# gduguey/DiffUS

Hardware: AMD Instinct MI355X
Metric: ray-steps/sec fwd+bwd (higher is better)
Workload: dtype f32

## Files before the change

### diffus_amd/csrc/scatter.hip

```cpp
#include "diffus_host.hpp"

namespace {

#ifdef DIFFUS_STAMP
__device__ unsigned long long *g_stamps = nullptr;
#define STAMP(i)                                                                          \
    do {                                                                                  \
        if (threadIdx.x == 0 && g_stamps) g_stamps[((size_t)blockIdx.y * gridDim.x + blockIdx.x) * 8 + (i)] = __builtin_readcyclecounter(); \
    } while (0)
#define STAMPV(i, v)                                                                     \
    do {                                                                                  \
        if (threadIdx.x == 0 && g_stamps) g_stamps[((size_t)blockIdx.y * gridDim.x + blockIdx.x) * 8 + (i)] = (unsigned long long)(v); \
    } while (0)
#define STAMP_NOW() __builtin_readcyclecounter()
#else
#define STAMP(i) ((void)0)
#define STAMPV(i, v) ((void)0)
#define STAMP_NOW() 0ull
#endif

template <int LAYOUT>
__device__ __forceinline__ int tile_unit(int v, int axis)
{
    if (LAYOUT == DIFFUS_CANONICAL) return v;
    return axis == 2 ? (v >> 1) : (v >> 2);
}

#ifndef DIFFUS_SCATTER_THREADS
#define DIFFUS_SCATTER_THREADS 256
#endif
#ifndef DIFFUS_SC_PATCH_STEPS
#define DIFFUS_SC_PATCH_STEPS DIFFUS_PATCH_STEPS
#endif
#ifndef DIFFUS_SC_PATCH_RAYS
#define DIFFUS_SC_PATCH_RAYS DIFFUS_PATCH_RAYS
#endif
#ifndef DIFFUS_SC_MIN_BLOCKS
#define DIFFUS_SC_MIN_BLOCKS 6
#endif
#ifdef DIFFUS_SC_EXIT
#define SC_EXIT(n)                                                                                                      \
    if (DIFFUS_SC_EXIT == (n)) {                                                                                        \
        _Pragma("unroll") for (int q_ = 0; q_ < kSPT; ++q_)                                                             \
            asm volatile("" ::"v"(zb[q_]), "v"(tx[q_]), "v"(ty[q_]), "v"(x0[q_]), "v"(y0[q_]), "v"(x1[q_]), "v"(y1[q_])); \
        return true;                                                                                                    \
    }
#else
#define SC_EXIT(n) ((void)0)
#endif
constexpr int kScRays = DIFFUS_SC_PATCH_RAYS, kScSteps = DIFFUS_SC_PATCH_STEPS;
constexpr int kSB = DIFFUS_SCATTER_THREADS, kSW = kSB / kWave, kSPT = kScRays * kScSteps / kSB;
#ifndef DIFFUS_SLAB_CAP
#define DIFFUS_SLAB_CAP 9216
#endif
#ifndef DIFFUS_SLAB_MIN_BLOCKS
#define DIFFUS_SLAB_MIN_BLOCKS 4
#endif
constexpr int kSlabCap = DIFFUS_SLAB_CAP;
#ifndef DIFFUS_SC_ROW_PAD
#define DIFFUS_SC_ROW_PAD 1
#endif
constexpr unsigned kRowPad = DIFFUS_SC_ROW_PAD;

template <int SAMPLER, int PM, int CAP>
__device__ __forceinline__ bool scatter_patch_planar(const Args &A, double *tile, int (*s_box)[4], int *s_planar, int *s_live, const Pose &ps,
                                                     const float *rows, unsigned row_off, bool ray_ok, int nbase, int tid)
{
    const int wib = tid >> 6;
    constexpr int kCapD = CAP / 2;
    float zb[kSPT];
    {
        const char *rb = reinterpret_cast<const char *>(rows);
#ifdef DIFFUS_ABLATE_SC_LOAD
        if (true) {
#pragma unroll
            for (int q = 0; q < kSPT; ++q) zb[q] = (ray_ok && nbase + q < A.N1) ? 1e-3f * (float)((tid + q) & 15) : 0.f;
        } else
#endif
        if (ray_ok && nbase + kSPT <= A.N1) {
            if constexpr (kSPT == 4) {
                const F4a4 t = *reinterpret_cast<const F4a4 *>(rb + (size_t)row_off);
                zb[0] = t.x; zb[1] = t.y; zb[2] = t.z; zb[3] = t.w;
            } else {
#pragma unroll
                for (int q = 0; q < kSPT; ++q) zb[q] = ldb_f32(rows, row_off + 4u * q);
            }
        } else {
#pragma unroll
            for (int q = 0; q < kSPT; ++q) zb[q] = (ray_ok && nbase + q < A.N1) ? ldb_f32(rows, row_off + 4u * q) : 0.f;
        }
    }
    {
        int4 *t4 = reinterpret_cast<int4 *>(tile);
#pragma unroll
        for (int e = 0; e < CAP / 4 / kSB; ++e) t4[e * kSB + tid] = make_int4(0, 0, 0, 0);
        static_assert(CAP % (4 * kSB) == 0, "tile clear assumes whole int4 passes");
    }
    const bool ray_planar = (PM == 0 || ps.pmode != 2) ? (ps.df[2] == 0.f) : (ps.dd[2] == 0.0);
    const bool wave_planar = __ballot(ray_planar) == ~0ull;
    int x0[kSPT], x1[kSPT], y0[kSPT], y1[kSPT];
    float tx[kSPT], ty[kSPT];
#pragma unroll
    for (int q = 0; q < kSPT; ++q) {
        const float kf = (float)(A.start + nbase + q);
        const float p0 = ray_point_f<PM>(ps, 0, kf), p1 = ray_point_f<PM>(ps, 1, kf);
        if (SAMPLER == DIFFUS_NEAREST) {
            x0[q] = x1[q] = nearest_index(p0, A.G.d0);
            y0[q] = y1[q] = nearest_index(p1, A.G.d1);
            tx[q] = ty[q] = 0.f;
        } else {
            const Axis a = tri_axis(p0, A.G.d0), b = tri_axis(p1, A.G.d1);
            x0[q] = a.i0; x1[q] = a.i1; tx[q] = a.t;
            y0[q] = b.i0; y1[q] = b.i1; ty[q] = b.t;
        }
    }
    const bool has = ray_ok && nbase < A.N1;
    int bx[4];
    bx[0] = has ? min(x0[0], x0[kSPT - 1]) : 0x7fffffff;
    bx[1] = has ? max(x1[0], x1[kSPT - 1]) : -1;
    bx[2] = has ? min(y0[0], y0[kSPT - 1]) : 0x7fffffff;
    bx[3] = has ? max(y1[0], y1[kSPT - 1]) : -1;
    if (tid == 0) *s_live = 0;
    STAMP(1);
    SC_EXIT(1);
    bx[0] = wave_reduce_minmax<true>(bx[0]);
    bx[1] = wave_reduce_minmax<false>(bx[1]);
    bx[2] = wave_reduce_minmax<true>(bx[2]);
    bx[3] = wave_reduce_minmax<false>(bx[3]);
    if ((tid & 63) == 63) {
        s_planar[wib] = wave_planar;
#pragma unroll
        for (int a = 0; a < 4; ++a) s_box[wib][a] = bx[a];
    }
    __syncthreads();
    STAMP(2);
    SC_EXIT(2);
    int wb[kSW][4];
    int all_planar = 1;
#pragma unroll
    for (int wv = 0; wv < kSW; ++wv) {
        all_planar &= s_planar[wv];
#pragma unroll
        for (int a = 0; a < 4; ++a) wb[wv][a] = __builtin_amdgcn_readfirstlane(s_box[wv][a]) >> 2;
    }
    if (!__builtin_amdgcn_readfirstlane(all_planar)) return false;
    auto box_of = [&](int w0, int cnt, int &l0, int &l1, int &b0, int &b1) -> int {
        int mn0 = 0x7fffffff, mx0 = -1, mn1 = 0x7fffffff, mx1 = -1;
#pragma unroll
        for (int wv = 0; wv < kSW; ++wv) {
            const bool in = wv >= w0 && wv < w0 + cnt;
            mn0 = in ? min(mn0, wb[wv][0]) : mn0; mx0 = in ? max(mx0, wb[wv][1]) : mx0;
            mn1 = in ? min(mn1, wb[wv][2]) : mn1; mx1 = in ? max(mx1, wb[wv][3]) : mx1;
        }
        l0 = mn0; l1 = mn1; b0 = mx0 - mn0 + 1; b1 = mx1 - mn1 + 1;
        if (mx0 < 0 || mx1 < 0) return 0;
        const unsigned e0 = (unsigned)min(b0, 0x3fff), e1 = (unsigned)min(b1, 0x3fff);
        return (int)min(4u * e0 * (4u * e1 + kRowPad), (unsigned)kCapD + 1u);
    };
    static_assert(kSW == 4 || kSW == 8, "wave grouping below: 1, 2 or 4 groups of waves");
    int nsub = 1, l0, l1, b0, b1;
    int need = box_of(0, kSW, l0, l1, b0, b1);
    if (need > kCapD) {
        int t0, t1, t2, t3;
        nsub = 2;
        if (box_of(0, kSW / 2, t0, t1, t2, t3) > kCapD || box_of(kSW / 2, kSW / 2, t0, t1, t2, t3) > kCapD) nsub = 4;
    }
    int iz0, iz1;
    float tz;
    {
        const float p2 = ray_point_f<PM>(ps, 2, 0.f);
        if (SAMPLER == DIFFUS_NEAREST) {
            iz0 = iz1 = nearest_index(p2, A.G.d2);
            tz = 0.f;
        } else {
            const Axis c = tri_axis(p2, A.G.d2);
            iz0 = c.i0; iz1 = c.i1; tz = c.t;
        }
        iz0 = __builtin_amdgcn_readfirstlane(iz0); iz1 = __builtin_amdgcn_readfirstlane(iz1);
        tz = __int_as_float(__builtin_amdgcn_readfirstlane(__float_as_int(tz)));
    }
    const int wpg = kSW / nsub;
    {
        unsigned nz = 0;
#pragma unroll
        for (int q = 0; q < kSPT; ++q) {
            if (!finitef(zb[q])) zb[q] = 0.f;
            nz |= __float_as_uint(zb[q]) & 0x7fffffffu;
        }
        if (__builtin_amdgcn_ballot_w64(nz != 0u) != 0ull && (tid & 63) == 63) *s_live = 1;
    }
#pragma unroll 1
    for (int sp = 0; sp < nsub; ++sp) {
        if (nsub > 1) need = box_of(sp * wpg, wpg, l0, l1, b0, b1);
        if (need == 0) continue;
        const bool mine = (wib / wpg) == sp;
#pragma unroll
        for (int q = 0; q < kSPT; ++q)
            asm volatile("" : "+v"(zb[q]), "+v"(tx[q]), "+v"(ty[q]), "+v"(x0[q]), "+v"(y0[q]), "+v"(x1[q]), "+v"(y1[q]));
        if (need > kCapD) {
            if (mine) {
#pragma unroll
                for (int q = 0; q < kSPT; ++q)
                    if (zb[q] != 0.f) {
                        Cell c;
                        c.i0[0] = x0[q]; c.i1[0] = x1[q]; c.t[0] = tx[q];
                        c.i0[1] = y0[q]; c.i1[1] = y1[q]; c.t[1] = ty[q];
                        c.i0[2] = iz0; c.i1[2] = iz1; c.t[2] = tz;
                        for_each_corner<SAMPLER>(c, zb[q], [&](int i, int j, int k, float v) {
                            if (v != 0.f) {
                                unsigned g = vox_off<DIFFUS_BRICKED>(A.G, i, j, k);
                                atomicAdd(A.gvol + g, v);
                                if (A.gtouched) A.gtouched[g >> 5] = 1;
                            }
                        });
                    }
            }
            continue;
        }
        STAMP(3);
    SC_EXIT(3);
        const int BY = 4 * b1 + kRowPad;
        const int org = -(4 * l0) * BY - 4 * l1;
        const int BY8 = BY * 8, org8 = org * 8;
        char *tile_c = reinterpret_cast<char *>(tile);
        auto add_at = [&](int byte_off, double v) { atomicAdd(reinterpret_cast<double *>(tile_c + byte_off), v); };
        if (mine) {
#pragma unroll
        for (int q = 0; q < kSPT; ++q) {
            const bool on = zb[q] != 0.f;
            const int r0 = __mul24(x0[q], BY8) + org8, r1 = __mul24(x1[q], BY8) + org8;
            const int e00 = r0 + 8 * y0[q], e11 = r1 + 8 * y1[q];
            float c00, c01 = 0.f, c10 = 0.f, c11 = 0.f;
            if constexpr (SAMPLER == DIFFUS_NEAREST) {
                c00 = zb[q];
            } else {
                const float wa1 = tx[q], wa0 = 1.f - wa1, wb1 = ty[q], wb0 = 1.f - wb1;
                const float s0 = zb[q] * wa0, s1 = zb[q] * wa1;
                c00 = s0 * wb0; c01 = s0 * wb1; c10 = s1 * wb0; c11 = s1 * wb1;
            }
#ifdef DIFFUS_ABLATE_SC_ADD
            asm volatile("" :: "v"(c00), "v"(c01), "v"(c10), "v"(c11), "v"(e00), "v"(e11));
            continue;
#endif
            const unsigned long long act = __builtin_amdgcn_ballot_w64(on);
            if (act == 0ull) continue;
            const int lead = __builtin_ctzll(act);
            const int f00 = __builtin_amdgcn_readlane(e00, lead), f11 = __builtin_amdgcn_readlane(e11, lead);
            const unsigned long long eq = __builtin_amdgcn_ballot_w64(e00 == f00) & __builtin_amdgcn_ballot_w64(e11 == f11);
            const bool same = (eq & act) == act;
            if (same && __builtin_popcountll(act) > 4) {
                const int f01 = __builtin_amdgcn_readlane(r0 + 8 * y1[q], lead), f10 = __builtin_amdgcn_readlane(r1 + 8 * y0[q], lead);
                const double t00 = wave_sum_to_lane63((double)c00);
                double t01 = 0.0, t10 = 0.0, t11 = 0.0;
                if constexpr (SAMPLER != DIFFUS_NEAREST) {
                    t01 = wave_sum_to_lane63((double)c01);
                    t10 = wave_sum_to_lane63((double)c10);
                    t11 = wave_sum_to_lane63((double)c11);
                }
                if ((tid & 63) == 63) {
                    if (t00 != 0.0) add_at(f00, t00);
                    if (t01 != 0.0) add_at(f01, t01);
                    if (t10 != 0.0) add_at(f10, t10);
                    if (t11 != 0.0) add_at(f11, t11);
                }
            } else {
                if (c00 != 0.f) add_at(e00, (double)c00);
                if constexpr (SAMPLER != DIFFUS_NEAREST) {
                    if (c01 != 0.f) add_at(r0 + 8 * y1[q], (double)c01);
                    if (c10 != 0.f) add_at(r1 + 8 * y0[q], (double)c10);
                    if (c11 != 0.f) add_at(e11, (double)c11);
                }
            }
            __builtin_amdgcn_sched_barrier(0);
        }
        }
        __syncthreads();
        STAMP(4);
    SC_EXIT(4);
        if (__builtin_amdgcn_readfirstlane(*s_live) == 0) continue;
        {
            const int lane = tid & 63, o = lane & 31, h = lane >> 5;
            const int zz = (o & 1) ? iz1 : iz0;
            const float wz = (iz1 == iz0) ? ((o & 1) ? 0.f : 1.f) : ((o & 1) ? tz : 1.f - tz);
            const bool adds = wz != 0.f, h0 = h == 0;
            const unsigned lc_tile = (unsigned)((__mul24(o >> 3, BY) + 4 * h + ((o >> 1) & 3)) * 8);
            const unsigned lc_g = (__umul24((unsigned)h, (unsigned)A.G.nb2) + (unsigned)(zz >> 1)) * kBrickFloats * 4u
                                  + (unsigned)(((o >> 1) << 1) + (zz & 1)) * 4u;
            const unsigned lc_t = (__umul24((unsigned)h, (unsigned)A.G.nb2) + (unsigned)(zz >> 1)) * 4u;
            unsigned lc_tile_o = lc_tile;
            asm volatile("" : "+v"(lc_tile_o));
            const char *tile_b = reinterpret_cast<const char *>(tile);
            const int wv = __builtin_amdgcn_readfirstlane(wib);
            const unsigned nb2u = (unsigned)A.G.nb2;
            char *const gvol_b = reinterpret_cast<char *>(A.gvol);
            char *const gt_b = reinterpret_cast<char *>(A.gtouched);
            auto flush_pair = [&](unsigned trow, unsigned grow, int cp, double &v, unsigned &ta) {
                const bool second = 2 * cp + 1 < b1;
                ta = trow + 64u * (unsigned)cp + lc_tile_o;
                v = (h0 || second) ? *reinterpret_cast<const double *>(tile_b + ta) : 0.0;
                (void)grow;
            };
            auto emit_pair = [&](unsigned grow, int cp, double v, unsigned ta) {
                if (nsub > 1 && v != 0.0 && !(o & 1)) *reinterpret_cast<double *>(const_cast<char *>(tile_b) + ta) = 0.0;
                const bool nz = v != 0.0 && adds;
#ifdef DIFFUS_ABLATE_SC_FLUSH
                asm volatile("" :: "s"(grow), "v"((float)v * wz), "v"(nz));
#else
                if (nz) {
                    const unsigned gb = grow + 2u * (unsigned)cp * nb2u;
                    if (A.gtouched) *reinterpret_cast<int *>(gt_b + (size_t)gb * 4u + (size_t)lc_t) = 1;
                    atomicAdd(reinterpret_cast<float *>(gvol_b + (size_t)gb * (kBrickFloats * 4u) + (size_t)lc_g), (float)v * wz);
                }
#endif
            };
            const int npr = (b1 + 1) >> 1;
            for (int ci = wv >> 1; ci < b0; ci += 2) {
                const unsigned trow = (unsigned)(4 * ci * BY) * 8u;
                const unsigned grow = ((unsigned)(l0 + ci) * (unsigned)A.G.nb1 + (unsigned)l1) * nb2u;
                for (int cp = wv & 1; cp < npr; cp += 4) {
                    double v0, v1 = 0.0;
                    unsigned t0, t1 = 0;
                    const bool two = cp + 2 < npr;
                    flush_pair(trow, grow, cp, v0, t0);
                    if (two) flush_pair(trow, grow, cp + 2, v1, t1);
                    emit_pair(grow, cp, v0, t0);
                    if (two) emit_pair(grow, cp + 2, v1, t1);
                }
            }
        }
        STAMP(5);
#ifdef DIFFUS_STAMP
        if (threadIdx.x == 0 && g_stamps) {
            g_stamps[((size_t)blockIdx.y * gridDim.x + blockIdx.x) * 8 + 6] = (unsigned long long)need;
            g_stamps[((size_t)blockIdx.y * gridDim.x + blockIdx.x) * 8 + 7] = (unsigned long long)nsub;
        }
#endif
        if (sp + 1 < nsub) __syncthreads();
    }
    return true;
}


template <int SAMPLER, int PM, int CAP>
__device__ __forceinline__ void scatter_patch_planar_merged(const Args &A, double *tile, int (*s_box)[4], int *s_planar, int *s_live, const Pose &ps,
                                                            const float *rows, unsigned row_off, bool ray_ok, int nbase, int ng, int tid)
{
    constexpr int kCapD = CAP / 2, kMaxG = 4;
    const int wib = tid >> 6;
    float zb[kMaxG][kSPT];
    {
        const char *rb = reinterpret_cast<const char *>(rows);
#pragma unroll
        for (int g = 0; g < kMaxG; ++g) {
            const int n0 = nbase + g * kScSteps;
            const unsigned off = row_off + (unsigned)(g * kScSteps) * 4u;
            if (g < ng && ray_ok && n0 + kSPT <= A.N1) {
                if constexpr (kSPT == 4) {
                    const F4a4 t = *reinterpret_cast<const F4a4 *>(rb + (size_t)off);
                    zb[g][0] = t.x; zb[g][1] = t.y; zb[g][2] = t.z; zb[g][3] = t.w;
                } else {
#pragma unroll
                    for (int q = 0; q < kSPT; ++q) zb[g][q] = ldb_f32(rows, off + 4u * q);
                }
            } else {
#pragma unroll
                for (int q = 0; q < kSPT; ++q) zb[g][q] = (g < ng && ray_ok && n0 + q < A.N1) ? ldb_f32(rows, off + 4u * q) : 0.f;
            }
        }
    }
    {
        int4 *t4 = reinterpret_cast<int4 *>(tile);
#pragma unroll
        for (int e = 0; e < CAP / 4 / kSB; ++e) t4[e * kSB + tid] = make_int4(0, 0, 0, 0);
    }
    const bool ray_planar = (PM == 0 || ps.pmode != 2) ? (ps.df[2] == 0.f) : (ps.dd[2] == 0.0);
    const bool wave_planar = __ballot(ray_planar) == ~0ull;
    auto cell_xy = [&](int n, int &x0, int &x1, int &y0, int &y1, float &tx, float &ty) {
        const float kf = (float)(A.start + n);
        const float p0 = ray_point_f<PM>(ps, 0, kf), p1 = ray_point_f<PM>(ps, 1, kf);
        if (SAMPLER == DIFFUS_NEAREST) {
            x0 = x1 = nearest_index(p0, A.G.d0); y0 = y1 = nearest_index(p1, A.G.d1);
            tx = ty = 0.f;
        } else {
            const Axis a = tri_axis(p0, A.G.d0), b = tri_axis(p1, A.G.d1);
            x0 = a.i0; x1 = a.i1; tx = a.t; y0 = b.i0; y1 = b.i1; ty = b.t;
        }
    };
    int bx[4];
    {
        int ax0, ax1, ay0, ay1, bx0, bx1, by0, by1;
        float t0, t1;
        cell_xy(nbase, ax0, ax1, ay0, ay1, t0, t1);
        cell_xy(nbase + (ng - 1) * kScSteps + kSPT - 1, bx0, bx1, by0, by1, t0, t1);
        const bool has = ray_ok && nbase < A.N1;
        bx[0] = has ? min(ax0, bx0) : 0x7fffffff; bx[1] = has ? max(ax1, bx1) : -1;
        bx[2] = has ? min(ay0, by0) : 0x7fffffff; bx[3] = has ? max(ay1, by1) : -1;
    }
    if (tid == 0) *s_live = 0;
    bx[0] = wave_reduce_minmax<true>(bx[0]);
    bx[1] = wave_reduce_minmax<false>(bx[1]);
    bx[2] = wave_reduce_minmax<true>(bx[2]);
    bx[3] = wave_reduce_minmax<false>(bx[3]);
    if ((tid & 63) == 63) {
        s_planar[wib] = wave_planar;
#pragma unroll
        for (int a = 0; a < 4; ++a) s_box[wib][a] = bx[a];
    }
    __syncthreads();
    int all_planar = 1, mn0 = 0x7fffffff, mx0 = -1, mn1 = 0x7fffffff, mx1 = -1;
#pragma unroll
    for (int wv = 0; wv < kSW; ++wv) {
        all_planar &= s_planar[wv];
        mn0 = min(mn0, __builtin_amdgcn_readfirstlane(s_box[wv][0]) >> 2); mx0 = max(mx0, __builtin_amdgcn_readfirstlane(s_box[wv][1]) >> 2);
        mn1 = min(mn1, __builtin_amdgcn_readfirstlane(s_box[wv][2]) >> 2); mx1 = max(mx1, __builtin_amdgcn_readfirstlane(s_box[wv][3]) >> 2);
    }
    if (mx0 < 0 || mx1 < 0) return;
    const int l0 = mn0, l1 = mn1, b0 = mx0 - mn0 + 1, b1 = mx1 - mn1 + 1;
    const unsigned need = min(4u * (unsigned)min(b0, 0x3fff) * (4u * (unsigned)min(b1, 0x3fff) + kRowPad), (unsigned)kCapD + 1u);
    if (!__builtin_amdgcn_readfirstlane(all_planar) || need > (unsigned)kCapD) {
#pragma unroll 1
// ... 476 lines not shown
            }
            bx[0] = wave_reduce_minmax<true>(any ? ulo : 0x7fffffff);
            bx[1] = wave_reduce_minmax<false>(any ? uhi : -1);
            bx[2] = wave_reduce_minmax<true>(any ? vlo : 0x7fffffff);
            bx[3] = wave_reduce_minmax<false>(any ? vhi : -1);
        }
        if ((tid & 63) == 63) {
#pragma unroll
            for (int a = 0; a < 4; ++a) s_rec[wib][2 + 4 * c + a] = bx[a];
        }
    }
    const int devbits = wave_reduce_minmax<false>(__float_as_int(dev));
    if ((tid & 63) == 63) {
        s_rec[wib][0] = (int)present;
        s_rec[wib][1] = devbits;
    }
    __syncthreads();
    present = 0;
    int dmax = 0;
    {
        int rp[kSW], rd[kSW];
#pragma unroll
        for (int wv = 0; wv < kSW; ++wv) { rp[wv] = s_rec[wv][0]; rd[wv] = s_rec[wv][1]; }
#pragma unroll
        for (int wv = 0; wv < kSW; ++wv) {
            present |= (unsigned)__builtin_amdgcn_readfirstlane(rp[wv]);
            dmax = max(dmax, __builtin_amdgcn_readfirstlane(rd[wv]));
        }
    }
    if (present == 0u) return true;
    int L = 2;
    float c0b = 0.f;
    if (present & 1u) {
        const float devmax = __int_as_float(dmax);
        const float dU = (float)(axU == 0 ? dims[0] : (axU == 1 ? dims[1] : dims[2])), dV = (float)(axV == 0 ? dims[0] : (axV == 1 ? dims[1] : dims[2]));
        const float T = fabsf(c0) + fabsf(cu) * dU + fabsf(cv) * dV + 2.f;
        const float S = fabsf(cu) + fabsf(cv) + devmax + (1e-4f + T * 0x1p-19f);
        if (!(S < 0.5f * (float)(kSlabMaxL - 2))) return false;
        L = (int)ceilf(2.f * S) + 2;
        c0b = c0 - S;
    }
    SLAB_EXIT(3, "s"(L), "s"(c0b), "v"(cls), "v"(sm[0].i0[0]), "v"(sm[1].i0[1]), "v"(sm[2].i0[2]), "v"(sm[3].i1[0]), "v"(sm[3].t[0]));
#ifdef DIFFUS_STAMP
    const unsigned long long t_rec = STAMP_NOW();
#endif
    STAMP(6);
    unsigned long long prof[5] = {0ull, 0ull, 0ull, 0ull, 0ull};
    const unsigned last_class = (present & 1u) ? ((present >> (ax + 2)) ? (31u - (unsigned)__builtin_clz(present)) : 0u)
                                               : (31u - (unsigned)__builtin_clz(present));
    auto run_pass = [&](auto axis_, auto face_) {
        constexpr int a = decltype(axis_)::value;
        constexpr bool face = decltype(face_)::value;
        const unsigned want = face ? (unsigned)(a + 1) : 0u;
        unsigned member = 0;
#pragma unroll
        for (int q = 0; q < kSPT; ++q) member |= ((((cls >> (2 * q)) & 3u) == want && zb[q] != 0.f) ? 1u : 0u) << q;
        int rb[kSW][4];
#pragma unroll
        for (int wv = 0; wv < kSW; ++wv)
#pragma unroll
            for (int e = 0; e < 4; ++e) rb[wv][e] = s_rec[wv][2 + 4 * want + e];
        int u0 = 0x7fffffff, u1 = -1, v0 = 0x7fffffff, v1 = -1;
#pragma unroll
        for (int wv = 0; wv < kSW; ++wv) {
            u0 = min(u0, __builtin_amdgcn_readfirstlane(rb[wv][0])); u1 = max(u1, __builtin_amdgcn_readfirstlane(rb[wv][1]));
            v0 = min(v0, __builtin_amdgcn_readfirstlane(rb[wv][2])); v1 = max(v1, __builtin_amdgcn_readfirstlane(rb[wv][3]));
        }
        slab_pass<SAMPLER, a, face, CAPD>(A, tile, sm, zb, member, cu, cv, c0b, face ? 2 : L, u0, u1, v0, v1, want == last_class, tid, prof);
    };
    using T_ = std::true_type;
    using F_ = std::false_type;
    if (present >> 1 & 1u) run_pass(std::integral_constant<int, 0>{}, T_{});
    if ((present & 1u) && ax == 0) run_pass(std::integral_constant<int, 0>{}, F_{});
    if (present >> 2 & 1u) run_pass(std::integral_constant<int, 1>{}, T_{});
    if ((present & 1u) && ax == 1) run_pass(std::integral_constant<int, 1>{}, F_{});
    if (present >> 3 & 1u) run_pass(std::integral_constant<int, 2>{}, T_{});
    if ((present & 1u) && ax == 2) run_pass(std::integral_constant<int, 2>{}, F_{});
#ifdef DIFFUS_STAMP
    STAMPV(3, prof[0]); STAMPV(4, prof[1]); STAMP(5); STAMPV(7, ((prof[3] * 16ull + prof[2]) << 24) | ((prof[4] - t_rec) & 0xffffffull));
#endif
    return true;
}

template <int SAMPLER, int LAYOUT, int PM, bool SLAB = false>
__global__ __launch_bounds__(kSB, SLAB ? DIFFUS_SLAB_MIN_BLOCKS : DIFFUS_SC_MIN_BLOCKS) void scatter_patch_kernel(Args A, int ray_groups, int has_finish, int step_groups, int sg_mul)
{
    constexpr int CAP = SLAB ? kSlabCap : kTileCap;
    static_assert(!SLAB || LAYOUT == DIFFUS_BRICKED, "the slab path scatters into a bricked gradient");
    __shared__ __attribute__((aligned(16))) int tile[CAP];
    __shared__ int s_slab[SLAB ? kSW : 1][18];
    __shared__ int s_wlo[kSW][3], s_whi[kSW][3];
    __shared__ float s_sum[kSW];
    __shared__ int s_planar[kSW];
    __shared__ int s_box[kSW][4];
    __shared__ int s_live;
    constexpr int UNIT = (LAYOUT == DIFFUS_CANONICAL) ? 1 : kBrickFloats;
    constexpr bool kCanPlanar = (LAYOUT == DIFFUS_BRICKED);

    if (has_finish && blockIdx.y == 0) {
        if (blockIdx.x < (unsigned)A.P) pose_finish_block<SAMPLER, LAYOUT, false>(A, (int)blockIdx.x, reinterpret_cast<float *>(tile));
        return;
    }
    const int tid = threadIdx.x;
    int pose, nbase, sg_blk = 0;
    bool ray_ok;
    long w, w0;
    unsigned row_off;
    auto decode = [&](unsigned bx, unsigned by) {
        const unsigned Lb = xcd_remap(bx, gridDim.x);
        const int rg = Lb % ray_groups;
        pose = Lb / ray_groups;
        const int row = (int)by - has_finish;
        const int sg = (int)(((unsigned)row * (unsigned)sg_mul + 3u * (unsigned)pose) % (unsigned)step_groups);
        sg_blk = sg;
        const int rl = tid / (kScSteps / kSPT);
        nbase = sg * kScSteps + (tid % (kScSteps / kSPT)) * kSPT;
        ray_ok = rg * kScRays + rl < A.R;
        w0 = (long)pose * A.R + (long)rg * kScRays;
        w = w0 + (ray_ok ? rl : 0);
        row_off = (__umul24((unsigned)(ray_ok ? rl : 0), (unsigned)A.N1) + (unsigned)nbase) * 4u;
    };
    unsigned bx = blockIdx.x, by = blockIdx.y;
#ifdef DIFFUS_SC_EXIT
    if (DIFFUS_SC_EXIT == 0) return;
#endif
    if (xcd_remap(bx, gridDim.x) >= (unsigned)A.P * (unsigned)ray_groups) return;
    decode(bx, by);

    STAMP(0);
#ifdef DIFFUS_SC_SALU_PAD
    {
        int pad = 0;
        asm volatile(".rept %1\n s_add_u32 %0, %0, 1\n .endr" : "+s"(pad) : "n"(DIFFUS_SC_SALU_PAD));
        asm volatile("" :: "s"(pad));
    }
#endif
#ifdef DIFFUS_SC_VALU_PAD
    {
        int pad = tid;
        asm volatile(".rept %1\n v_add_u32 %0, %0, 1\n .endr" : "+v"(pad) : "n"(DIFFUS_SC_VALU_PAD));
        asm volatile("" :: "v"(pad));
    }
#endif
    Pose ps;
    if constexpr (PM == 0) {
        const float *sp = (const float *)A.src + (long)pose * 3, *dp = (const float *)A.dirs + w0 * 3;
        const unsigned doff = (unsigned)(w - w0) * 12u;
#pragma unroll
        for (int c = 0; c < 3; ++c) {
            ps.sf[c] = sp[c];
            ps.df[c] = ldb_f32(dp, doff + 4u * c);
        }
        ps.pmode = 0;
    } else {
        load_pose<PM>(ps, A.src, A.src_f64, A.dirs, A.dir_f64, pose, w);
    }
#ifndef DIFFUS_SC_MERGE
#define DIFFUS_SC_MERGE 1
#endif
    if constexpr (kCanPlanar && !SLAB && PM == 0 && DIFFUS_SC_MERGE > 1) {
        if (A.fans_planar) {
            const float *sp = (const float *)A.src + (long)pose * 3;
            const int nr = min(kScRays, A.R - (int)(w0 - (long)pose * A.R));
            const float *da = (const float *)A.dirs + w0 * 3, *db = (const float *)A.dirs + (w0 + nr - 1) * 3;
            const float hx = (float)(A.G.d0 - 1), hy = (float)(A.G.d1 - 1);
            auto outside = [&](int sgq) -> bool {
                const float kf = (float)(A.start + sgq * kScSteps);
                const float ax = __fadd_rn(sp[0], __fmul_rn(kf, da[0])), ay = __fadd_rn(sp[1], __fmul_rn(kf, da[1]));
                const float bxp = __fadd_rn(sp[0], __fmul_rn(kf, db[0])), byp = __fadd_rn(sp[1], __fmul_rn(kf, db[1]));
                const bool oa = !(ax > 0.f && ax < hx && ay > 0.f && ay < hy), ob = !(bxp > 0.f && bxp < hx && byp > 0.f && byp < hy);
                return oa && ob;
            };
            if (__builtin_amdgcn_readfirstlane((int)outside(sg_blk))) {
                constexpr int kMg = DIFFUS_SC_MERGE;
                const bool leader = (sg_blk & (kMg - 1)) == 0 || !__builtin_amdgcn_readfirstlane((int)outside(sg_blk - 1));
                if (!leader) return;
                const int lim = min(kMg - (sg_blk & (kMg - 1)), step_groups - sg_blk);
                int ng = 1;
                while (ng < lim && __builtin_amdgcn_readfirstlane((int)outside(sg_blk + ng))) ++ng;
                if (ng > 1) {
                    scatter_patch_planar_merged<SAMPLER, PM, CAP>(A, reinterpret_cast<double *>(tile), s_box, s_planar, &s_live, ps, A.zbar + w0 * A.N1,
                                                                  row_off, ray_ok, nbase, ng, tid);
                    return;
                }
            }
        }
    }
    if constexpr (kCanPlanar) {
        bool try_planar = true;
        float dfl[6], zpre[kSPT];
        if constexpr (SLAB) {
            const long wl = w0 + (long)min(kScRays, A.R - (int)(w0 - (long)pose * A.R)) - 1;
#pragma unroll
            for (int q = 0; q < kSPT; ++q) zpre[q] = (ray_ok && nbase + q < A.N1) ? ldb_f32(A.zbar + w0 * A.N1, row_off + 4u * q) : 0.f;
#pragma unroll
            for (int c = 0; c < 3; ++c) {
                dfl[c] = A.dir_f64 ? (float)((const double *)A.dirs)[w0 * 3 + c] : ((const float *)A.dirs)[w0 * 3 + c];
                dfl[3 + c] = A.dir_f64 ? (float)((const double *)A.dirs)[wl * 3 + c] : ((const float *)A.dirs)[wl * 3 + c];
            }
            try_planar = __builtin_amdgcn_readfirstlane((int)(dfl[2] == 0.f)) != 0;
        }
        if (try_planar) {
        if (scatter_patch_planar<SAMPLER, PM, CAP>(A, reinterpret_cast<double *>(tile), s_box, s_planar, &s_live, ps, A.zbar + w0 * A.N1, row_off, ray_ok, nbase, tid)) return;
#ifdef DIFFUS_SC_PLANAR_ONLY
        return;
#endif
        __syncthreads();
        asm volatile("" : "+s"(bx), "+s"(by));
        decode(bx, by);
        load_pose<PM>(ps, A.src, A.src_f64, A.dirs, A.dir_f64, pose, w);
        } else {
            int4 *t4 = reinterpret_cast<int4 *>(tile);
#pragma unroll
            for (int e = 0; e < CAP / 4 / kSB; ++e) t4[e * kSB + tid] = make_int4(0, 0, 0, 0);
        }
        if constexpr (SLAB) {
            if (scatter_patch_slab<SAMPLER, PM, CAP>(A, reinterpret_cast<double *>(tile), s_slab, ps, dfl, zpre, nbase, tid)) return;
            __syncthreads();
            asm volatile("" : "+s"(bx), "+s"(by));
            decode(bx, by);
            load_pose<PM>(ps, A.src, A.src_f64, A.dirs, A.dir_f64, pose, w);
        }
    }
    Cell cells[kSPT];
    float zb[kSPT];
    int lo[3] = {0x7fffffff, 0x7fffffff, 0x7fffffff}, hi[3] = {-1, -1, -1};
#pragma unroll
    for (int q = 0; q < kSPT; ++q) {
        int n = nbase + q;
        zb[q] = 0.f;
        if (ray_ok && n < A.N1) zb[q] = A.zbar[w * A.N1 + n];
    }
    {
        int4 *t4 = reinterpret_cast<int4 *>(tile);
#pragma unroll
        for (int e = 0; e < CAP / 4 / kSB; ++e) t4[e * kSB + tid] = make_int4(0, 0, 0, 0);
        static_assert(CAP % (4 * kSB) == 0, "tile clear assumes whole int4 passes");
    }
#pragma unroll
    for (int q = 0; q < kSPT; ++q) cells[q] = cell_of<SAMPLER, PM>(A, ps, A.start + nbase + q);
    float zsum = 0.f;
#pragma unroll
    for (int q = 0; q < kSPT; ++q) {
        if (!finitef(zb[q])) zb[q] = 0.f;
        zsum += fabsf(zb[q]);
        if (zb[q] != 0.f) {
#pragma unroll
            for (int a = 0; a < 3; ++a) {
                lo[a] = min(lo[a], tile_unit<LAYOUT>(cells[q].i0[a], a));
                hi[a] = max(hi[a], tile_unit<LAYOUT>(cells[q].i1[a], a));
            }
        }
    }
    STAMP(1);
#pragma unroll
    for (int a = 0; a < 3; ++a) {
        lo[a] = wave_reduce_minmax<true>(lo[a]);
        hi[a] = wave_reduce_minmax<false>(hi[a]);
    }
    zsum = wave_sum_to_lane63(zsum);
    const int wib = tid >> 6;
    if ((tid & 63) == 63) {
#pragma unroll
        for (int a = 0; a < 3; ++a) {
            s_wlo[wib][a] = lo[a];
            s_whi[wib][a] = hi[a];
        }
        s_sum[wib] = zsum;
    }
    __syncthreads();
    STAMP(2);
    int wlo[kSW][3], whi[kSW][3];
#pragma unroll
    for (int wv = 0; wv < kSW; ++wv)
#pragma unroll
        for (int a = 0; a < 3; ++a) {
            wlo[wv][a] = __builtin_amdgcn_readfirstlane(s_wlo[wv][a]);
            whi[wv][a] = __builtin_amdgcn_readfirstlane(s_whi[wv][a]);
        }
    auto box_of = [&](int w0, int cnt, int (&l)[3], int (&b)[3]) -> int {
        unsigned v = UNIT;
        bool empty = false;
#pragma unroll
        for (int a = 0; a < 3; ++a) {
            int mn = 0x7fffffff, mx = -1;
#pragma unroll
            for (int wv = 0; wv < kSW; ++wv) {
                const bool in = wv >= w0 && wv < w0 + cnt;
                mn = in ? min(mn, wlo[wv][a]) : mn;
                mx = in ? max(mx, whi[wv][a]) : mx;
            }
            l[a] = mn;
            b[a] = mx - mn + 1;
            empty |= mx < 0;
            const unsigned e = (unsigned)min(max(b[a], 0), 0x7fff);
            v = min(v, (unsigned)CAP + 1u) * e;
        }
        return empty ? 0 : (int)min(v, (unsigned)CAP + 1u);
    };
    static_assert(kSW == 4 || kSW == 8, "wave grouping below: 1, 2 or 4 groups of waves");
    int nsub = 1;
    int lb[3], bb[3];
    int vol_tile = box_of(0, kSW, lb, bb);
    if (vol_tile > CAP) {
        int l[3], b[3];
        nsub = 2;
// ... 33 lines not shown
    const int l0 = lb[0], l1 = lb[1], l2 = lb[2], b0 = bb[0], b1 = bb[1], b2 = bb[2];
    const int nt = vol_tile;
    STAMP(3);
    auto part = [&](int v, int axis) -> int {
        if (LAYOUT == DIFFUS_CANONICAL)
            return axis == 0 ? (v - l0) * b1 * b2 : (axis == 1 ? (v - l1) * b2 : (v - l2));
        return axis == 0 ? (((v >> 2) - l0) * b1 * b2 * kBrickFloats + ((v & 3) << 3))
                         : (axis == 1 ? (((v >> 2) - l1) * b2 * kBrickFloats + ((v & 3) << 1))
                                      : (((v >> 1) - l2) * kBrickFloats + (v & 1)));
    };
#pragma unroll
    for (int q = 0; q < kSPT; ++q)
        if (mine && zb[q] != 0.f) {
            const Cell &c = cells[q];
            const float sc = ldexpf(zb[q], fx);
            if (SAMPLER == DIFFUS_NEAREST) {
                atomicAdd(&tile[part(c.i0[0], 0) + part(c.i0[1], 1) + part(c.i0[2], 2)], __float2int_rn(sc));
            } else {
                const int ex0 = part(c.i0[0], 0), ex1 = part(c.i1[0], 0), ey0 = part(c.i0[1], 1), ey1 = part(c.i1[1], 1),
                          ez0 = part(c.i0[2], 2), ez1 = part(c.i1[2], 2);
                const float wa1 = c.t[0], wa0 = 1.f - wa1, wb1 = c.t[1], wb0 = 1.f - wb1, wc1 = c.t[2], wc0 = 1.f - wc1;
                const float w00 = sc * wa0 * wb0, w01 = sc * wa0 * wb1, w10 = sc * wa1 * wb0, w11 = sc * wa1 * wb1;
                auto add = [&](int e, float v) {
                    int q = __float2int_rn(v);
                    if (q != 0) atomicAdd(&tile[e], q);
                };
                add(ex0 + ey0 + ez0, w00 * wc0);
                add(ex0 + ey0 + ez1, w00 * wc1);
                add(ex0 + ey1 + ez0, w01 * wc0);
                add(ex0 + ey1 + ez1, w01 * wc1);
                add(ex1 + ey0 + ez0, w10 * wc0);
                add(ex1 + ey0 + ez1, w10 * wc1);
                add(ex1 + ey1 + ez0, w11 * wc0);
                add(ex1 + ey1 + ez1, w11 * wc1);
            }
        }
    __syncthreads();
    STAMP(4);
    const int b12 = b1 * b2, nunits = b0 * b12;
    const float rb2 = __frcp_rn((float)b2), rb12 = __frcp_rn((float)b12);
    constexpr int LPU = (UNIT == 1) ? 1 : UNIT;
    const int o = (UNIT == 1) ? 0 : (tid & (LPU - 1));
    const int msub = tid / LPU, mstep = kSB / LPU;
    constexpr int FU = 4;
    for (int q0 = msub; q0 < nunits; q0 += mstep * FU) {
        int v[FU];
#pragma unroll
        for (int u = 0; u < FU; ++u) {
            const int q = q0 + u * mstep;
            v[u] = (q < nunits) ? tile[q * UNIT + o] : 0;
            if (nsub > 1 && v[u] != 0) tile[q * UNIT + o] = 0;
        }
#pragma unroll
        for (int u = 0; u < FU; ++u) {
            const int q = q0 + u * mstep;
            bool any = v[u] != 0;
            if (UNIT != 1) any = (unsigned)(__ballot(v[u] != 0) >> (tid & 32)) != 0u;
            if (any) {
                const int i = __float2int_rz(((float)q + 0.5f) * rb12);
                const int m = q - i * b12;
                const int j = __float2int_rz(((float)m + 0.5f) * rb2);
                const int k = m - j * b2;
                unsigned g;
                if (LAYOUT == DIFFUS_CANONICAL)
                    g = ((unsigned)(l0 + i) * (unsigned)A.G.d1 + (unsigned)(l1 + j)) * (unsigned)A.G.d2 + (unsigned)(l2 + k);
                else
                    g = (((unsigned)(l0 + i) * (unsigned)A.G.nb1 + (unsigned)(l1 + j)) * (unsigned)A.G.nb2 + (unsigned)(l2 + k)) * kBrickFloats + (unsigned)o;
                if (LAYOUT == DIFFUS_BRICKED && A.gtouched && o == 0) A.gtouched[g >> 5] = 1;
                if (v[u] != 0) atomicAdd(A.gvol + g, ldexpf((float)v[u], -fx));
            }
        }
    }
    STAMP(5);
#ifdef DIFFUS_STAMP
    if (threadIdx.x == 0 && g_stamps) {
        g_stamps[((size_t)blockIdx.y * gridDim.x + blockIdx.x) * 8 + 6] = (unsigned long long)nt;
        g_stamps[((size_t)blockIdx.y * gridDim.x + blockIdx.x) * 8 + 7] = (unsigned long long)nsub;
    }
#endif
    if (sp + 1 < nsub) __syncthreads();
    }
}

}

namespace diffus {
int launch_scatter(const Args &A, int sampler, int layout, hipStream_t st)
{
    const int rgs = (A.R + kScRays - 1) / kScRays, sgs = (A.N1 + kScSteps - 1) / kScSteps;
    int sg_mul = 1;
    if (sgs >= 3) {
        auto gcd = [](int a, int b) { while (b) { const int t = a % b; a = b; b = t; } return a; };
        sg_mul = ((sgs * 7) / 16) | 1;
        while (sg_mul < sgs && gcd(sg_mul, sgs) != 1) sg_mul += 2;
        if (sg_mul >= sgs) sg_mul = 1;
    }
    const int fin = A.finish_in_scatter ? 1 : 0;
    const dim3 grid((unsigned)((((long)A.P * rgs + 7) / 8) * 8), (unsigned)(sgs + fin));
    const bool f32 = !A.src_f64 && !A.dir_f64;
    const int glayout = layout == DIFFUS_PAIRED ? DIFFUS_BRICKED : layout;
    return dispatch_sl(sampler, glayout, [&](auto S_, auto L_) {
        constexpr int SM = decltype(S_)::value, LY = (decltype(L_)::value == DIFFUS_PAIRED) ? DIFFUS_BRICKED : decltype(L_)::value;
        if constexpr (LY == DIFFUS_BRICKED) {
            if (!A.fans_planar) {
                if (f32)
                    hipLaunchKernelGGL((scatter_patch_kernel<SM, LY, 0, true>), grid, dim3(kSB), 0, st, A, rgs, fin, sgs, sg_mul);
                else
                    hipLaunchKernelGGL((scatter_patch_kernel<SM, LY, 1, true>), grid, dim3(kSB), 0, st, A, rgs, fin, sgs, sg_mul);
                return last_launch();
            }
        }
        if (f32)
            hipLaunchKernelGGL((scatter_patch_kernel<SM, LY, 0>), grid, dim3(kSB), 0, st, A, rgs, fin, sgs, sg_mul);
        else
            hipLaunchKernelGGL((scatter_patch_kernel<SM, LY, 1>), grid, dim3(kSB), 0, st, A, rgs, fin, sgs, sg_mul);
        return last_launch();
    });
}
}

namespace {

constexpr int kConvZ = 64, kConvZThin = 8;
template <bool TO_BRICKED, bool ACCUMULATE, int CZ = kConvZ>
__global__ __launch_bounds__(kBlock) void brick_convert_kernel(const float *__restrict__ in, float *__restrict__ out,
                                                               Geom G, int zblk0 = 0, int by_0 = 0, int bx_0 = 0)
{
    __shared__ float t[16][CZ + 1];
    const int bz0 = ((int)blockIdx.x + zblk0) * (CZ / 2);
    const int by = blockIdx.y + by_0, bx = blockIdx.z + bx_0;
    const int tid = threadIdx.x;
    const long brick0 = ((long)bx * G.nb1 + by) * G.nb2 + bz0;
    if (TO_BRICKED) {
        for (int e = tid; e < 16 * CZ; e += kBlock) {
            int row = e / CZ, zz = e - row * CZ;
            int x = bx * 4 + (row >> 2), y = by * 4 + (row & 3), z = bz0 * 2 + zz;
            t[row][zz] = (x < G.d0 && y < G.d1 && z < G.d2) ? in[((long)x * G.d1 + y) * G.d2 + z] : 0.f;
        }
        __syncthreads();
        for (int e = tid; e < 16 * CZ; e += kBlock) {
            int brick = e >> 5, off = e & 31;
            if (bz0 + brick < G.nb2) out[(brick0 + brick) * kBrickFloats + off] = t[off >> 1][brick * 2 + (off & 1)];
        }
    } else {
        for (int e = tid; e < 16 * CZ; e += kBlock) {
            int brick = e >> 5, off = e & 31;
            if (bz0 + brick < G.nb2) t[off >> 1][brick * 2 + (off & 1)] = in[(brick0 + brick) * kBrickFloats + off];
        }
        __syncthreads();
        for (int e = tid; e < 16 * CZ; e += kBlock) {
            int row = e / CZ, zz = e - row * CZ;
            int x = bx * 4 + (row >> 2), y = by * 4 + (row & 3), z = bz0 * 2 + zz;
            if (x < G.d0 && y < G.d1 && z < G.d2) {
                long o = ((long)x * G.d1 + y) * G.d2 + z;
                if (ACCUMULATE)
                    out[o] += t[row][zz];
                else
                    out[o] = t[row][zz];
            }
        }
    }
}

__global__ __launch_bounds__(kBlock) void gradbuf_flush_dense_kernel(float *__restrict__ bricked, int *__restrict__ touched,
                                                                     float *__restrict__ out, Geom G, long nbricks)
{
    const int wib = threadIdx.x >> 6;
    const long w = (long)blockIdx.x * kWavesPerBlock + wib;
    const int lane = threadIdx.x & 63;
    const long b0 = w * kWave;
    if (b0 >= nbricks) return;
    const long mine = b0 + lane;
    int f = (mine < nbricks) ? touched[mine] : 0;
    {
        if (mine >= nbricks) return;
        if (f) touched[mine] = 0;
        const bool live = f == 1;
        const unsigned um = (unsigned)mine, t = um / (unsigned)G.nb2, bz = um - t * (unsigned)G.nb2;
        const unsigned bx = t / (unsigned)G.nb1, by = t - bx * (unsigned)G.nb1;
        float *bsrc = bricked + mine * kBrickFloats;
        const int z = (int)bz * 2;
#pragma unroll 4
        for (int row = 0; row < 16; ++row) {
            const int x = (int)bx * 4 + (row >> 2), y = (int)by * 4 + (row & 3);
            float2 v = make_float2(0.f, 0.f);
            if (live) {
                v = *reinterpret_cast<const float2 *>(bsrc + row * 2);
                *reinterpret_cast<float2 *>(bsrc + row * 2) = make_float2(0.f, 0.f);
            }
            if (x < G.d0 && y < G.d1) {
                float *o = out + ((long)x * G.d1 + y) * G.d2 + z;
// ... 232 lines not shown
```

Baseline: 77.14 billion.

## Add persistent walk kernel for planar scatter with zbar prefetch

Measured after the change: 60.56 billion (median of 6 runs). 0.785x the previous value.

```diff
diff --git a/diffus_amd/csrc/scatter.hip b/diffus_amd/csrc/scatter.hip
--- a/diffus_amd/csrc/scatter.hip
+++ b/diffus_amd/csrc/scatter.hip
@@ -1,4 +1,6 @@
 #include "diffus_host.hpp"
+#include <algorithm>
+#include <atomic>
 
 namespace {
 
@@ -62,14 +64,26 @@
 #endif
 constexpr unsigned kRowPad = DIFFUS_SC_ROW_PAD;
 
-template <int SAMPLER, int PM, int CAP>
+struct PlanarCol {
+    int wave_planar;
+    int iz0, iz1;
+    float tz;
+};
+struct NoPrefetch {
+    __device__ void operator()() const {}
+};
+template <int SAMPLER, int PM, int CAP, bool WALK = false, typename PF = NoPrefetch>
 __device__ __forceinline__ bool scatter_patch_planar(const Args &A, double *tile, int (*s_box)[4], int *s_planar, int *s_live, const Pose &ps,
-                                                     const float *rows, unsigned row_off, bool ray_ok, int nbase, int tid)
+                                                     const float *rows, unsigned row_off, bool ray_ok, int nbase, int tid,
+                                                     const PlanarCol *col = nullptr, const float *zin = nullptr, PF prefetch = PF())
 {
     const int wib = tid >> 6;
     constexpr int kCapD = CAP / 2;
     float zb[kSPT];
-    {
+    if constexpr (WALK) {
+#pragma unroll
+        for (int q = 0; q < kSPT; ++q) zb[q] = zin[q];
+    } else {
         const char *rb = reinterpret_cast<const char *>(rows);
 #ifdef DIFFUS_ABLATE_SC_LOAD
         if (true) {
@@ -90,14 +104,19 @@
             for (int q = 0; q < kSPT; ++q) zb[q] = (ray_ok && nbase + q < A.N1) ? ldb_f32(rows, row_off + 4u * q) : 0.f;
         }
     }
-    {
+    if constexpr (!WALK) {
         int4 *t4 = reinterpret_cast<int4 *>(tile);
 #pragma unroll
         for (int e = 0; e < CAP / 4 / kSB; ++e) t4[e * kSB + tid] = make_int4(0, 0, 0, 0);
         static_assert(CAP % (4 * kSB) == 0, "tile clear assumes whole int4 passes");
     }
-    const bool ray_planar = (PM == 0 || ps.pmode != 2) ? (ps.df[2] == 0.f) : (ps.dd[2] == 0.0);
-    const bool wave_planar = __ballot(ray_planar) == ~0ull;
+    bool wave_planar;
+    if constexpr (WALK) {
+        wave_planar = col->wave_planar != 0;
+    } else {
+        const bool ray_planar = (PM == 0 || ps.pmode != 2) ? (ps.df[2] == 0.f) : (ps.dd[2] == 0.0);
+        wave_planar = __ballot(ray_planar) == ~0ull;
+    }
     int x0[kSPT], x1[kSPT], y0[kSPT], y1[kSPT];
     float tx[kSPT], ty[kSPT];
 #pragma unroll
@@ -167,7 +186,9 @@
     }
     int iz0, iz1;
     float tz;
-    {
+    if constexpr (WALK) {
+        iz0 = col->iz0; iz1 = col->iz1; tz = col->tz;
+    } else {
         const float p2 = ray_point_f<PM>(ps, 2, 0.f);
         if (SAMPLER == DIFFUS_NEAREST) {
             iz0 = iz1 = nearest_index(p2, A.G.d2);
@@ -180,6 +201,7 @@
         tz = __int_as_float(__builtin_amdgcn_readfirstlane(__float_as_int(tz)));
     }
     const int wpg = kSW / nsub;
+    bool prefetched = false;
     {
         unsigned nz = 0;
 #pragma unroll
@@ -273,6 +295,12 @@
             }
             __builtin_amdgcn_sched_barrier(0);
         }
+        }
+        if constexpr (WALK) {
+            if (sp == nsub - 1) {
+                prefetch();
+                prefetched = true;
+            }
         }
         __syncthreads();
         STAMP(4);
@@ -301,7 +329,11 @@
                 (void)grow;
             };
             auto emit_pair = [&](unsigned grow, int cp, double v, unsigned ta) {
-                if (nsub > 1 && v != 0.0 && !(o & 1)) *reinterpret_cast<double *>(const_cast<char *>(tile_b) + ta) = 0.0;
+#ifdef DIFFUS_WALK_DIAG_NOZERO
+                if ((nsub > 1) && v != 0.0 && !(o & 1)) *reinterpret_cast<double *>(const_cast<char *>(tile_b) + ta) = 0.0;
+#else
+                if ((WALK || nsub > 1) && v != 0.0 && !(o & 1)) *reinterpret_cast<double *>(const_cast<char *>(tile_b) + ta) = 0.0;
+#endif
                 const bool nz = v != 0.0 && adds;
 #ifdef DIFFUS_ABLATE_SC_FLUSH
                 asm volatile("" :: "s"(grow), "v"((float)v * wz), "v"(nz));
@@ -336,6 +368,9 @@
         }
 #endif
         if (sp + 1 < nsub) __syncthreads();
+    }
+    if constexpr (WALK) {
+        if (!prefetched) prefetch();
     }
     return true;
 }
@@ -978,6 +1013,10 @@
     return true;
 }
 
+template <int SAMPLER, int LAYOUT, int PM, int CAP>
+__device__ __forceinline__ void scatter_patch_general(const Args &A, int *tile, int (*s_wlo)[3], int (*s_whi)[3], float *s_sum, const Pose &ps,
+                                                      long w, bool ray_ok, int nbase, int tid);
+
 template <int SAMPLER, int LAYOUT, int PM, bool SLAB = false>
 __global__ __launch_bounds__(kSB, SLAB ? DIFFUS_SLAB_MIN_BLOCKS : DIFFUS_SC_MIN_BLOCKS) void scatter_patch_kernel(Args A, int ray_groups, int has_finish, int step_groups, int sg_mul)
 {
@@ -990,7 +1029,6 @@
     __shared__ int s_planar[kSW];
     __shared__ int s_box[kSW][4];
     __shared__ int s_live;
-    constexpr int UNIT = (LAYOUT == DIFFUS_CANONICAL) ? 1 : kBrickFloats;
     constexpr bool kCanPlanar = (LAYOUT == DIFFUS_BRICKED);
 
     if (has_finish && blockIdx.y == 0) {
@@ -1118,6 +1156,14 @@
             load_pose<PM>(ps, A.src, A.src_f64, A.dirs, A.dir_f64, pose, w);
         }
     }
+    scatter_patch_general<SAMPLER, LAYOUT, PM, CAP>(A, tile, s_wlo, s_whi, s_sum, ps, w, ray_ok, nbase, tid);
+}
+
+template <int SAMPLER, int LAYOUT, int PM, int CAP>
+__device__ __forceinline__ void scatter_patch_general(const Args &A, int *tile, int (*s_wlo)[3], int (*s_whi)[3], float *s_sum, const Pose &ps,
+                                                      long w, bool ray_ok, int nbase, int tid)
+{
+    constexpr int UNIT = (LAYOUT == DIFFUS_CANONICAL) ? 1 : kBrickFloats;
     Cell cells[kSPT];
     float zb[kSPT];
     int lo[3] = {0x7fffffff, 0x7fffffff, 0x7fffffff}, hi[3] = {-1, -1, -1};
@@ -1317,6 +1363,180 @@
     }
 }
 
+template <int SAMPLER, int PM>
+__global__ __launch_bounds__(kSB, DIFFUS_SC_MIN_BLOCKS) void scatter_walk_kernel(Args A, int ray_groups, int has_finish, int step_groups, double per_block)
+{
+    constexpr int CAP = kTileCap;
+    __shared__ __attribute__((aligned(16))) int tile[CAP];
+    __shared__ int s_wlo[kSW][3], s_whi[kSW][3];
+    __shared__ float s_sum[kSW];
+    __shared__ int s_planar[2][kSW];
+    __shared__ int s_box[2][kSW][4];
+    __shared__ int s_live[2];
+    if (has_finish && blockIdx.y == 0) {
+        if (blockIdx.x < (unsigned)A.P) pose_finish_block<SAMPLER, DIFFUS_BRICKED, false>(A, (int)blockIdx.x, reinterpret_cast<float *>(tile));
+        return;
+    }
+    const int tid = threadIdx.x;
+    const unsigned nblk = gridDim.x, b = xcd_remap(blockIdx.x, nblk);
+    const unsigned T = (unsigned)A.P * (unsigned)ray_groups * (unsigned)step_groups;
+    unsigned p = (unsigned)__builtin_amdgcn_readfirstlane((int)(unsigned)((double)b * per_block));
+    unsigned pe = (b + 1 == nblk) ? T : (unsigned)__builtin_amdgcn_readfirstlane((int)(unsigned)((double)(b + 1) * per_block));
+    if (p >= pe) return;
+    {
+        int4 *t4 = reinterpret_cast<int4 *>(tile);
+#pragma unroll
+        for (int e = 0; e < CAP / 4 / kSB; ++e) t4[e * kSB + tid] = make_int4(0, 0, 0, 0);
+    }
+#define rl (tid / (kScSteps / kSPT))
+#define sl ((tid % (kScSteps / kSPT)) * kSPT)
+    const unsigned col0 = p / (unsigned)step_groups;
+    int sg = (int)(p - col0 * (unsigned)step_groups), rg = (int)(col0 % (unsigned)ray_groups), pose = (int)(col0 / (unsigned)ray_groups);
+#ifdef DIFFUS_WALK_DIAG_MIX
+    {
+        const unsigned nc = (unsigned)A.P * (unsigned)ray_groups, row = p / nc, c = p % nc;
+        pose = (int)(c / (unsigned)ray_groups); rg = (int)(c % (unsigned)ray_groups);
+        int m = 1;
+        if (step_groups >= 3) {
+            auto gcd = [](int a, int b2) { while (b2) { const int t = a % b2; a = b2; b2 = t; } return a; };
+            m = ((step_groups * 7) / 16) | 1;
+            while (m < step_groups && gcd(m, step_groups) != 1) m += 2;
+            if (m >= step_groups) m = 1;
+        }
+        sg = (int)((row * (unsigned)m + 3u * (unsigned)pose) % (unsigned)step_groups);
+        pe = p + 1;
+    }
+#endif
+    Pose ps;
+    PlanarCol pc;
+    bool ray_ok;
+    long w0;
+    auto load_pose_of = [&](Pose &q, int pose_, int rg_) {
+        const bool ok = rg_ * kScRays + rl < A.R;
+        const long c0 = (long)pose_ * A.R + (long)rg_ * kScRays;
+        if constexpr (PM == 0) {
+            const float *sp = (const float *)A.src + (long)pose_ * 3, *dp = (const float *)A.dirs + c0 * 3;
+            const unsigned doff = (unsigned)(ok ? rl : 0) * 12u;
+#pragma unroll
+            for (int c = 0; c < 3; ++c) {
+                q.sf[c] = sp[c];
+                q.df[c] = ldb_f32(dp, doff + 4u * c);
+            }
+            q.pmode = 0;
+        } else {
+            load_pose<PM>(q, A.src, A.src_f64, A.dirs, A.dir_f64, pose_, c0 + (ok ? rl : 0));
+        }
+    };
+    auto enter_column = [&]() {
+        ray_ok = rg * kScRays + rl < A.R;
+        w0 = (long)pose * A.R + (long)rg * kScRays;
+        load_pose_of(ps, pose, rg);
+        const bool ray_planar = (PM == 0 || ps.pmode != 2) ? (ps.df[2] == 0.f) : (ps.dd[2] == 0.0);
+        pc.wave_planar = __ballot(ray_planar) == ~0ull;
+        const float p2 = ray_point_f<PM>(ps, 2, 0.f);
+        int iz0, iz1;
+        float tz;
+        if (SAMPLER == DIFFUS_NEAREST) {
+            iz0 = iz1 = nearest_index(p2, A.G.d2);
+            tz = 0.f;
+        } else {
+            const Axis c = tri_axis(p2, A.G.d2);
+            iz0 = c.i0; iz1 = c.i1; tz = c.t;
+        }
+        pc.iz0 = __builtin_amdgcn_readfirstlane(iz0); pc.iz1 = __builtin_amdgcn_readfirstlane(iz1);
+        pc.tz = __int_as_float(__builtin_amdgcn_readfirstlane(__float_as_int(tz)));
+    };
+    auto load_zb = [&](float (&z)[kSPT], int pose_, int rg_, int s) {
+        const bool ok = rg_ * kScRays + rl < A.R;
+        const int c0 = __builtin_amdgcn_readfirstlane(pose_ * A.R + rg_ * kScRays);
+        const float *rows = A.zbar + (long)c0 * A.N1;
+        const int nb = s * kScSteps + sl;
+        const unsigned off = (__umul24((unsigned)(ok ? rl : 0), (unsigned)A.N1) + (unsigned)nb) * 4u;
+        if (ok && nb + kSPT <= A.N1) {
+            if constexpr (kSPT == 4) {
+                const F4a4 t = *reinterpret_cast<const F4a4 *>(reinterpret_cast<const char *>(rows) + (size_t)off);
+                z[0] = t.x; z[1] = t.y; z[2] = t.z; z[3] = t.w;
+            } else {
+#pragma unroll
+                for (int q = 0; q < kSPT; ++q) z[q] = ldb_f32(rows, off + 4u * q);
+            }
+        } else {
+#pragma unroll
+            for (int q = 0; q < kSPT; ++q) z[q] = (ok && nb + q < A.N1) ? ldb_f32(rows, off + 4u * q) : 0.f;
+        }
+    };
+    float zc[kSPT], zn[kSPT];
+    load_zb(zc, pose, rg, sg);
+    enter_column();
+#pragma unroll 1
+    for (int par = 0;; par ^= 1) {
+        const bool more = p + 1 < pe;
+        int sgn = sg + 1, rgn = rg, posen = pose;
+        if (sgn == step_groups) {
+            sgn = 0;
+            if (++rgn == ray_groups) { rgn = 0; ++posen; }
+        }
+        auto prefetch = [&]() {
+            if (more) {
+                load_zb(zn, posen, rgn, sgn);
+            }
+        };
+        const int nbase = sg * kScSteps + sl;
+        const unsigned row_off = (__umul24((unsigned)(ray_ok ? rl : 0), (unsigned)A.N1) + (unsigned)nbase) * 4u;
+        if (!scatter_patch_planar<SAMPLER, PM, CAP, true>(A, reinterpret_cast<double *>(tile), s_box[par], s_planar[par], &s_live[par], ps,
+                                                         A.zbar + w0 * A.N1, row_off, ray_ok, nbase, tid, &pc, zc, prefetch)) {
+            break;
+        }
+        if (!more) {
+            ++p;
+            break;
+        }
+        ++p;
+#pragma unroll
+        for (int q = 0; q < kSPT; ++q) zc[q] = zn[q];
+        const bool new_col = sgn == 0;
+        sg = sgn; rg = rgn; pose = posen;
+        if (new_col) {
+            enter_column();
+        } else {
+            load_pose_of(ps, pose, rg);
+        }
+    }
+    asm volatile("" : "+s"(p));
+#pragma unroll 1
+    for (; p < pe; ++p) {
+        __syncthreads();
+        const unsigned cq = p / (unsigned)step_groups;
+        const int sgq = (int)(p - cq * (unsigned)step_groups), rgq = (int)(cq % (unsigned)ray_groups), poseq = (int)(cq / (unsigned)ray_groups);
+        const bool okq = rgq * kScRays + rl < A.R;
+        Pose pg;
+        load_pose_of(pg, poseq, rgq);
+        scatter_patch_general<SAMPLER, DIFFUS_BRICKED, PM, CAP>(A, tile, s_wlo, s_whi, s_sum, pg, (long)poseq * A.R + (long)rgq * kScRays + (okq ? rl : 0), okq,
+                                                                sgq * kScSteps + sl, tid);
+    }
+}
+#undef rl
+#undef sl
+
+template <int SM, int PM>
+long walk_resident()
+{
+    constexpr int kMaxDev = 64;
+    static std::atomic<long> cache[kMaxDev];
+    int dev = 0;
+    if (hipGetDevice(&dev) != hipSuccess) dev = 0;
+    const int slot = (dev >= 0 && dev < kMaxDev) ? dev : 0;
+    long r = cache[slot].load(std::memory_order_relaxed);
+    if (r > 0) return r;
+    int cus = 256, per_cu = DIFFUS_SC_MIN_BLOCKS;
+    if (hipDeviceGetAttribute(&cus, hipDeviceAttributeMultiprocessorCount, dev) != hipSuccess || cus < 1) cus = 256;
+    if (hipOccupancyMaxActiveBlocksPerMultiprocessor(&per_cu, scatter_walk_kernel<SM, PM>, kSB, 0) != hipSuccess || per_cu < 1)
+        per_cu = DIFFUS_SC_MIN_BLOCKS;
+    r = (long)cus * per_cu;
+    cache[slot].store(r, std::memory_order_relaxed);
+    return r;
+}
+
 }
 
 namespace diffus {
@@ -1342,6 +1562,27 @@
                     hipLaunchKernelGGL((scatter_patch_kernel<SM, LY, 0, true>), grid, dim3(kSB), 0, st, A, rgs, fin, sgs, sg_mul);
                 else
                     hipLaunchKernelGGL((scatter_patch_kernel<SM, LY, 1, true>), grid, dim3(kSB), 0, st, A, rgs, fin, sgs, sg_mul);
+                return last_launch();
+            }
+            if constexpr (DIFFUS_SC_MERGE == 1) {
+                const long T = (long)A.P * rgs * sgs;
+                const long res = f32 ? walk_resident<SM, 0>() : walk_resident<SM, 1>();
+                long g = std::min(T, res - A.P);
+                g = (g >= T) ? (T + 7) / 8 * 8 : g / 8 * 8;
+#if defined(DIFFUS_WALK_DIAG_ONE) || defined(DIFFUS_WALK_DIAG_MIX)
+                g = (T + 7) / 8 * 8;
+#endif
+#ifdef DIFFUS_WALK_DIAG_TWO
+                g = std::min((T + 7) / 8 * 8, 2 * g);
+#endif
+                g = std::max(g, ((long)A.P + 7) / 8 * 8);
+                g = std::max(g, 8L);
+                const dim3 wgrid((unsigned)g, (unsigned)(1 + fin));
+                const double per_block = (double)T / (double)g;
+                if (f32)
+                    hipLaunchKernelGGL((scatter_walk_kernel<SM, 0>), wgrid, dim3(kSB), 0, st, A, rgs, fin, sgs, per_block);
+                else
+                    hipLaunchKernelGGL((scatter_walk_kernel<SM, 1>), wgrid, dim3(kSB), 0, st, A, rgs, fin, sgs, per_block);
                 return last_launch();
             }
         }
```
